# foges/pogs

Hardware: AMD Instinct MI355X
Metric: admm_iterations_per_sec_dense_lasso_fp32 (per-GPU shard, summed over GPUs) (higher is better)
Workload: dtype f32

## Files before the change

pogs_amd/csrc/dense_iter.h:

```cpp

template <typename T, typename Tag>
void DenseSolver<T, Tag>::load_problem(const FnHost &f, const FnHost &g, const SolveParams &p) {
  load_functions(f, g);
  bool all_cheap = true, all_logistic = true;
  if (tmode_) {
    all_logistic = false;
    all_cheap = all_h(g, n_, [](int h) { return is_cheap_prox(h); });
  } else {
    all_cheap = all_h(f, m_, [](int h) { return is_cheap_prox(h); });
    all_logistic = all_h(f, m_, [](int h) { return h == kLogistic; });
  }
  fused_now_ = fused_ok_ && (all_cheap || all_logistic);
  fused_logistic_ = fused_now_ && all_logistic && !all_cheap;
  tune_stream_plan<T>(planA_, fused_now_, fused_logistic_, tmode_);
  arm_control(p);
}

template <typename T, typename Tag>
void DenseSolver<T, Tag>::cold_start() {
  reset_iterate();
  spec_valid_ = false;
  exact_mode_ = false;
  colparts_ = 0;
  proj_count_ = 0;
}

template <typename T, typename Tag>
void DenseSolver<T, Tag>::apply_warm_start() {
  if (!warm_pending_) return;
  warm_pending_ = false;
  hipStream_t s = ctx_.stream;
  const T rho = ctl_.rho;
  POGS_HIP_CHECK(hipMemcpyAsync(xtemp_.p, warm_x_.data(), n_ * sizeof(T), hipMemcpyHostToDevice, s));
  POGS_HIP_CHECK(hipMemcpyAsync(ytemp_.p, warm_l_.data(), m_ * sizeof(T), hipMemcpyHostToDevice, s));
  launch_scale_by<T>(n_, static_cast<T>(1), xtemp_.p, e_.p, true, x_[cur_].p, s);
  launch_scale_by<T>(m_, static_cast<T>(1), ytemp_.p, d_.p, true, yt_.p, s);
  if (tmode_) {
    t_mul_n(x_[cur_].p, nullptr, GemvNOp<T>{1, 0, y_[cur_].p}, nullptr);
    t_mul_t(yt_.p, StoreColOp<T>{static_cast<T>(1) / rho, 0, xt_.p, n_}, nullptr);
  } else {
    StreamArgs<T> a = argsA();
    a.xin = x_[cur_].p;
    launch_stream<T, true, false, false, kFull, Tag>(planA_, a, GemvNOp<T>{1, 0, y_[cur_].p}, s);
    gemv_t_partials(yt_.p);
    finish_cols(StoreColOp<T>{static_cast<T>(1) / rho, 0, xt_.p, n_}, nullptr, 0, 0);
  }
  launch_scal<T>(yt_.p, static_cast<T>(-1) / rho, m_, s);
  ctx_.sync();
  xtemp_.zero(s);
  ytemp_.zero(s);
}

template <typename T, typename Tag>
bool DenseSolver<T, Tag>::iteration(unsigned verbose) {
  if (fused_now_) return tmode_ ? iteration_fused_wide(verbose) : iteration_fused(verbose);
  hipStream_t s = ctx_.stream;
  const int nw = cur_ ^ 1;
  const bool multi = multi_;
  const AdmmPreArgs<T> pa = pre_args();
  const double *S_fused = nullptr;
  if (cg_fused_) {
    S_fused = prox_and_project_fused(pa, nw);
  } else {
    launch_admm_pre<T>(pa, s);
    SumJob j[2] = {{ctx_.spart.p, pa.blocks_x, 3, ctx_.S.p + kGapX},
                   {ctx_.spart.p + static_cast<size_t>(pa.blocks_x) * 3, pre_blocks(m_), 3, ctx_.S.p + kGapY}};
    launch_sum_jobs(j, 2, s);
  }
  if (cg_fused_) {
  } else if (use_cgls_) {
    POGS_HIP_CHECK(hipMemcpyAsync(x_[nw].p, x_[cur_].p, n_ * sizeof(T), hipMemcpyDeviceToDevice, s));
    const bool ysync = ysync_ <= 0 || (proj_count_ % static_cast<unsigned long long>(ysync_)) == 0;
    ++proj_count_;
    const int steps = cgls_project(xtemp_.p, ytemp_.p, x_[nw].p, ctl_.proj_tol(), y_[cur_].p, ysync ? nullptr : y_[nw].p);
    if (ysync) {
      StreamArgs<T> a = argsA();
      a.xin = x_[nw].p;
      ctx_.stream_timer.begin(s);
      launch_stream<T, true, false, false, kFull, Tag>(planA_, a,
                                                  ProjTailOp<T>{y_[nw].p, y_[cur_].p, y12_.p, ytemp_.p}, s);
      ctx_.stream_timer.end(s);
      sum_row_scalars(stream_grid<true, false>(planA_, m_), 2, ctx_.S.p + kDYprev2);
      ctx_.stats.matvecs += 1;
    } else {
      if (steps == 0) POGS_HIP_CHECK(hipMemcpyAsync(y_[nw].p, y_[cur_].p, m_ * sizeof(T), hipMemcpyDeviceToDevice, s));
      double *spy = ctx_.spart.p;
      launch_admm_tail<T>(m_, y_[nw].p, y_[cur_].p, y12_.p, ytemp_.p, spy, s);
      SumJob jy{spy, vec_blocks(m_), 2, ctx_.S.p + kDYprev2};
      launch_sum_jobs(&jy, 1, s);
    }
    double *sp2 = ctx_.spart.p + static_cast<size_t>(planA_.grid_max) * 6;
    launch_admm_tail<T>(n_, x_[nw].p, x_[cur_].p, x12_.p, xtemp_.p, sp2, s);
    SumJob jt{sp2, vec_blocks(n_), 2, ctx_.S.p + kDXprev2};
    launch_sum_jobs(&jt, 1, s);
  } else if (tall_) {
    gemv_t_partials(ytemp_.p);
    finish_cols(StoreColOp<T>{1, 0, rhs_.p, n_}, nullptr, kGapY, 3);
    solve_gram_onepass(rhs_.p, xtemp_.p, ProjTailSumColOp<T>{x_[nw].p, x_[cur_].p, x12_.p, xtemp_.p, n_},
                       ctx_.S.p + kDXprev2);
    StreamArgs<T> a = argsA();
    a.xin = x_[nw].p;
    ctx_.stream_timer.begin(s);
    launch_stream<T, true, false, false, kFull, Tag>(planA_, a,
                                                ProjTailOp<T>{y_[nw].p, y_[cur_].p, y12_.p, ytemp_.p}, s);
    ctx_.stream_timer.end(s);
    sum_row_scalars(stream_grid<true, false>(planA_, m_), 2, ctx_.S.p + kDYprev2);
    if (multi) ctx_.dist.allreduce(ctx_.S.p + kDYprev2, 2, s);
  } else {
    t_mul_n(xtemp_.p, nullptr, ResidOp<T>{ytemp_.p, rhs_.p}, nullptr);
    solve_gram_onepass(rhs_.p, static_cast<const T *>(nullptr),
                       ProjTailAddColOp<T>{y_[nw].p, y_[cur_].p, y12_.p, ytemp_.p, tmpn_.p, m_},
                       ctx_.S.p + kDYprev2);
    t_mul_t(tmpn_.p, ProjTailColOp<T>{x_[nw].p, x_[cur_].p, x12_.p, xtemp_.p, n_}, ctx_.S.p + kDXprev2);
  }
  if (!use_cgls_) ctx_.stats.matvecs += 2;
  const double *S = S_fused ? S_fused : ctx_.fetch_scalars();
  ctl_.set_pre(S);
  bool exact = false;
  if (ctl_.set_approx(S, nrmA_)) {
    StreamArgs<T> a = argsA();
    const int grid = stream_grid<true, true>(planA_, srows_);
    if (tmode_) {
      launch_exact_u<T>(m_, y12_.p, yt_.p, y_[cur_].p, zt_scale_, uvec_.p, s);
      a.xin = uvec_.p;
      ctx_.stream_timer.begin(s);
      launch_stream<T, true, true, false, kFull, Tag>(planA_, a, ExactTRowOp<T>{x12_.p, xt_.p, x_[cur_].p, zt_scale_}, s);
      ctx_.stream_timer.end(s);
      sum_row_scalars(grid, 1, ctx_.S.p + kExactS2);
      double *sp = ctx_.spart.p + static_cast<size_t>(planA_.grid_max) * 6;
      launch_reduce_cols<T, ExactTColOp<T>>(colpart_.p, grid, scols_pad_, ExactTColOp<T>{y12_.p, m_}, sp, s);
      SumJob j{sp, reduce_cols_grid(scols_pad_, Vec16<T>::N), 1, ctx_.S.p + kExactR2};
      launch_sum_jobs(&j, 1, s);
    } else {
      a.xin = x12_.p;
      ctx_.stream_timer.begin(s);
      launch_stream<T, true, true, false, kFull, Tag>(planA_, a,
                                                 ExactRowOp<T>{y12_.p, yt_.p, y_[cur_].p, zt_scale_}, s);
      ctx_.stream_timer.end(s);
      sum_row_scalars(grid, 1, ctx_.S.p + kExactR2);
      finish_cols(ExactColOp<T>{x12_.p, xt_.p, x_[cur_].p, zt_scale_, n_}, ctx_.S.p + kExactS2, kExactR2, 1, grid);
    }
    ctx_.stats.matvecs += 1;
    S = ctx_.fetch_scalars();
    ctl_.set_exact(S);
    exact = true;
  }
  const bool stop = ctl_.check_stop(exact);
  log_iteration(verbose);
  if (stop) return true;
  advance(nw);
  return false;
}

template <typename T, typename Tag>
bool DenseSolver<T, Tag>::iteration_fused(unsigned verbose) {
  hipStream_t s = ctx_.stream;
  const int nw = cur_ ^ 1;
  const int by = pre_blocks(m_);
  const int gridC = pre_cols_grid(n_pad_, Vec16<T>::N);
  struct DeferGuard {
    bool &flag;
    DeferGuard(bool &f, bool on) : flag(f) { flag = on; }
    ~DeferGuard() { flag = false; }
  } defer_guard(defer_sums_, true);
  const bool spec = spec_valid_;
  double *pre_part = ctx_.spart.p + sp_pre_off_;
  double *pc_part = pre_part + static_cast<size_t>(by) * 3;
  double *tail = pack_.p ? pack_.p + 2 * static_cast<size_t>(n_pad_) : nullptr;
  const size_t pack_count = 2 * static_cast<size_t>(n_pad_) + 6;
#ifndef POGS_LEAN_F32_NV5
#define POGS_LEAN_F32_NV5 0
#endif
  constexpr bool kLeanType = std::is_same<T, double>::value || (POGS_LEAN_F32_NV5 != 0 && Tag::has(256, 5) && !Tag::windows);
  const bool lean = kLeanType && !multi_ && !exact_mode_ && !mixed_full_;
  int nparts = colparts_ > 0 ? colparts_ : stream2_grid<2>(planA_, m_);
  if (!spec) {
    AdmmPreArgs<T> pa = pre_args();
    pa.n_x = 0;
    pa.partials = pre_part;
    pa.blocks_x = 0;
    launch_admm_pre<T>(pa, s);
    const SumJob jy{pre_part, by, 3, ctx_.S.p + kGapY};
    StreamArgs2<T> a2{A_.p, lda_, m_, n_pad_, nullptr, nullptr, colpart_.p, colpart2_.p, ctx_.spart.p};
    ctx_.stream_timer.begin(s);
    launch_stream2<T, 0, 2, Tag>(planA_, a2, PreAccOp<T>{ytemp_.p, y12_.p, yt_.p, y_[cur_].p, zt_scale_}, s);
    ctx_.stream_timer.end(s);
    nparts = stream2_grid<0>(planA_, m_);
    ctx_.stats.matvecs += 1;
    if (!multi_) {
      sum_now_or_later(jy);
    } else {
      PackJobs pj;
      pj.j[0] = jy; pj.j[1] = jy; pj.njobs = 1;
      launch_pack_cols<T>(colpart_.p, colpart2_.p, nparts, n_pad_, pack_.p, pj, s);
      ctx_.dist.allreduce(pack_.p, pack_count, s);
      ScalarOverlay ov;
      ov.src = tail; ov.slot[0] = kGapY; ov.n[0] = 3;
      launch_apply_overlay(ctx_.S.p, ov, s);
    }
  }
  {
    PreColsArgs<T> pc;
    pc.part0 = colpart_.p; pc.part1 = (lean && spec) ? nullptr : colpart2_.p; pc.nparts = nparts;
    pc.tot64 = pack_.p;
    pc.n = n_; pc.n_pad = n_pad_;
    pc.g = gview();
    pc.x_cur = x_[cur_].p; pc.xt = xt_.p;
    pc.zt_scale = zt_scale_; pc.rho = ctl_.rho; pc.alpha = ctl_.alpha();
    pc.x12 = x12_.p; pc.xtemp = xtemp_.p; pc.rhs = rhs_.p;
    pc.partials = pc_part;
    launch_pre_cols<T>(pc, multi_, s);
    sum_now_or_later(SumJob{pc_part, gridC, 3, ctx_.S.p + kGapX, 4, 0});
    sum_now_or_later(SumJob{pc_part, gridC, 1, ctx_.S.p + kExactS2, 4, 3});
  }
  solve_gram_onepass(rhs_.p, xtemp_.p, ProjTailSumColOp<T>{x_[nw].p, x_[cur_].p, x12_.p, xtemp_.p, n_},
                     ctx_.S.p + kDXprev2);
  {
    StreamArgs2<T> a2{A_.p, lda_, m_, n_pad_, x_[nw].p, x12_.p, colpart_.p, colpart2_.p, ctx_.spart.p};
    ctl_.predict(&rho_pred_, &zs_pred_);
    const bool timed = ctx_.stream_timer.begin(s) != EventTimer::npos;
    int grid = stream2_grid<2>(planA_, m_);
    bool mixed_done = false;
    if constexpr (std::is_same<T, double>::value) {
      if (mixed_pass_) {
        const StreamArgsMixed am{A32_.p, lda32_, m_, n_pad_, static_cast<int>(lda32_), x_[nw].p, x12_.p, colpart_.p, colpart2_.p,
                                 ctx_.spart.p};
        if (fused_logistic_) {
          launch_stream2_mixed(planM_, !lean, am, FusedIterOp<double, true>{y_[nw].p, y_[cur_].p, y12_.p, ytemp_.p, fview(), rho_pred_,
                                                                            ctl_.alpha(), zs_pred_, y12s_.p, ytemps_.p}, s);
        } else {
          launch_stream2_mixed(planM_, !lean, am, FusedIterOp<double, false>{y_[nw].p, y_[cur_].p, y12_.p, ytemp_.p, fview(), rho_pred_,
                                                                             ctl_.alpha(), zs_pred_, y12s_.p, ytemps_.p}, s);
        }
        grid = mixed_grid(planM_, !lean, m_);
        if (timed) ++mixed_timed_;
        mixed_done = true;
      }
    }
    if (mixed_done) {
    } else if (fused_logistic_) {
      FusedIterOp<T, true> op{y_[nw].p, y_[cur_].p, y12_.p, ytemp_.p, fview(), rho_pred_, ctl_.alpha(), zs_pred_,
                              y12s_.p, ytemps_.p};
      if constexpr (kLeanType) {
        if (lean) { launch_stream2<T, 1, 1, Tag>(planA_, a2, op, s); grid = stream2_grid<1, 1>(planA_, m_); }
        else launch_stream2<T, 2, 2, Tag>(planA_, a2, op, s);
      } else {
        launch_stream2<T, 2, 2, Tag>(planA_, a2, op, s);
      }
    } else {
      FusedIterOp<T, false> op{y_[nw].p, y_[cur_].p, y12_.p, ytemp_.p, fview(), rho_pred_, ctl_.alpha(), zs_pred_,
                               y12s_.p, ytemps_.p};
      if constexpr (kLeanType) {
        if (lean) { launch_stream2<T, 1, 1, Tag>(planA_, a2, op, s); grid = stream2_grid<1, 1>(planA_, m_); }
        else launch_stream2<T, 2, 2, Tag>(planA_, a2, op, s);
      } else {
        launch_stream2<T, 2, 2, Tag>(planA_, a2, op, s);
      }
    }
    ctx_.stream_timer.end(s);
    colparts_ = grid;
    const SumJob jd{ctx_.spart.p, grid, 3, ctx_.S.p + kDYprev2, 6, 0};
    const SumJob js{ctx_.spart.p, grid, 3, ctx_.S.p + kSpecGapY, 6, 3};
    if (!multi_) {
      sum_now_or_later(jd);
      sum_now_or_later(js);
    } else {
      PackJobs pj;
      pj.j[0] = jd; pj.j[1] = js; pj.njobs = 2;
      launch_pack_cols<T>(colpart_.p, colpart2_.p, grid, n_pad_, pack_.p, pj, s);
      ctx_.dist.allreduce(pack_.p, pack_count, s);
      ScalarOverlay ov;
      ov.src = tail;
      ov.slot[0] = kDYprev2; ov.n[0] = 3;
      ov.slot[1] = kSpecGapY; ov.n[1] = 3;
      ctx_.set_overlay(ov);
    }
    ctx_.stats.matvecs += 1;
  }
  double S[kNumSlots];
  std::memcpy(S, ctx_.fetch_scalars(), sizeof(S));
  if (spec)
    for (int q = 0; q < 3; ++q) S[kGapY + q] = spec_gap_[q];
  ctl_.set_pre(S);
  bool exact = false;
  bool drop_spec = false;
  if (ctl_.set_approx(S, nrmA_)) {
    if (lean) {
      StreamArgs<T> a = argsA();
      a.xin = x12_.p;
      a.col_partials = colpart2_.p;
      const int g1 = stream_grid<true, true>(planA_, srows_);
      ctx_.stream_timer.begin(s);
      launch_stream<T, true, true, false, kFull, Tag>(planA_, a, ExactRowOp<T>{y12_.p, yt_.p, y_[cur_].p, zt_scale_}, s);
      ctx_.stream_timer.end(s);
      sum_row_scalars(g1, 1, ctx_.S.p + kExactR2);
      finish_cols(ExactColOp<T>{x12_.p, xt_.p, x_[cur_].p, zt_scale_, n_}, ctx_.S.p + kExactS2, kExactR2, 1, g1, colpart2_.p);
      ctx_.stats.matvecs += 1;
      const double *S2 = ctx_.fetch_scalars();
      S[kExactR2] = S2[kExactR2];
      S[kExactS2] = S2[kExactS2];
      exact_mode_ = true;
      drop_spec = true;
    }
    ctl_.set_exact(S);
    exact = true;
  }
  const bool stop = ctl_.check_stop(exact);
  log_iteration(verbose);
  if (stop) return true;
  advance(nw);
  if (!drop_spec && ctl_.rho == rho_pred_ && zt_scale_ == zs_pred_) {
    std::swap(ytemp_, ytemps_);
    std::swap(y12_, y12s_);
    for (int q = 0; q < 3; ++q) spec_gap_[q] = S[kSpecGapY + q];
    spec_valid_ = true;
    ctx_.stats.reserved[0] += 1;
  } else {
    spec_valid_ = false;
    ctx_.stats.reserved[1] += 1;
  }
  return false;
}

template <typename T, typename Tag>
void DenseSolver<T, Tag>::collect_timer() {
  const unsigned long long cnt = collect_timer_head();
  const unsigned long long mixed = std::min(mixed_timed_, cnt);
  mixed_timed_ = 0;
  ctx_.stats.stream_bytes += static_cast<double>(cnt - mixed) * m_ * n_ * sizeof(T) + static_cast<double>(mixed) * m_ * n_ * sizeof(float);
}
```

pogs_amd/csrc/dense_setup.h:

```cpp

template <typename T, typename Tag>
void DenseSolver<T, Tag>::upload(int ord, const void *A, int mem) {
  hipStream_t s = ctx_.stream;
  A_.alloc(static_cast<size_t>(srows_) * lda_);
  const hipMemcpyKind kind = (mem == POGS_AMD_DEVICE) ? hipMemcpyDeviceToDevice : hipMemcpyHostToDevice;
  const char *ae = std::getenv("POGS_AMD_ALIAS_INPUT");
  bool may_alias = mem == POGS_AMD_DEVICE && !(ae && ae[0] == '0') &&
                   (reinterpret_cast<uintptr_t>(A) % 16) == 0;
  if (may_alias) {
    hipPointerAttribute_t attr;
    if (hipPointerGetAttributes(&attr, A) != hipSuccess) {
      (void)hipGetLastError();
      may_alias = false;
    } else {
      may_alias = attr.type == hipMemoryTypeDevice && attr.device == ctx_.device;
    }
  }
  if (tmode_) {
    if (lda_ != static_cast<size_t>(m_)) A_.zero(s);
    if (ord != ROW_MAJ && may_alias && lda_ == static_cast<size_t>(m_)) {
      A_src_ = static_cast<const T *>(A);
    } else if (ord != ROW_MAJ) {
      POGS_HIP_CHECK(hipMemcpy2DAsync(A_.p, lda_ * sizeof(T), A, m_ * sizeof(T), m_ * sizeof(T), n_, kind, s));
    } else {
      DevBuf<T> stage;
      const T *src = static_cast<const T *>(A);
      if (mem != POGS_AMD_DEVICE) {
        stage.alloc(static_cast<size_t>(m_) * n_);
        POGS_HIP_CHECK(hipMemcpyAsync(stage.p, A, static_cast<size_t>(m_) * n_ * sizeof(T), kind, s));
        src = stage.p;
      }
      launch_transpose<T>(src, n_, m_, n_, A_.p, lda_, s);
      ctx_.sync();
    }
  } else if (ord == ROW_MAJ && may_alias && lda_ == static_cast<size_t>(n_)) {
    A_src_ = static_cast<const T *>(A);
  } else if (ord == ROW_MAJ) {
    if (lda_ != static_cast<size_t>(n_)) A_.zero(s);
    POGS_HIP_CHECK(hipMemcpy2DAsync(A_.p, lda_ * sizeof(T), A, n_ * sizeof(T), n_ * sizeof(T), m_, kind, s));
  } else {
    DevBuf<T> stage;
    const T *src = static_cast<const T *>(A);
    if (mem != POGS_AMD_DEVICE) {
      stage.alloc(static_cast<size_t>(m_) * n_);
      POGS_HIP_CHECK(hipMemcpyAsync(stage.p, A, static_cast<size_t>(m_) * n_ * sizeof(T), kind, s));
      src = stage.p;
    }
    if (lda_ != static_cast<size_t>(n_)) A_.zero(s);
    launch_transpose<T>(src, m_, n_, m_, A_.p, lda_, s);
    ctx_.sync();
  }
  ctx_.sync();
}

template <typename T, typename Tag>
void DenseSolver<T, Tag>::alloc_state() {
  hipStream_t s = ctx_.stream;
  const size_t np = n_pad_;
  const size_t mp = m_pad_;
  alloc_iterate(np, mp);
  const size_t kp = std::max<size_t>(np, k_pad_);
  rhs_.alloc(kp); tvec_.alloc(kp); tmpn_.alloc(kp);
  rhs_.zero(s); tvec_.zero(s); tmpn_.zero(s);
  d_.zero(s); e_.zero(s);
  if (tmode_) { uvec_.alloc(mp); uvec_.zero(s); }
  const size_t gmax = std::max<size_t>(planA_.grid_max, mixed_store_ ? mixed_grid_max(planM_) : 0);
  colpart_.alloc(gmax * scols_pad_);
  ensure_xl(planA_, srows_, scols_pad_);
  if (use_cgls_) {
    cg_p_.alloc(np); cg_s_.alloc(np); cg_q_.alloc(m_); cg_r_.alloc(m_); cg_.alloc(kCgNumSlots);
    cg_p_.zero(s); cg_s_.zero(s); cg_.zero(s);
    if (cg_fused_) alloc_cg_fused();
  }
  const char *fe = std::getenv("POGS_AMD_FUSED");
  fused_ok_ = (tall_ || tmode_) && !use_cgls_ && stream2_supported(planA_) && !(fe && fe[0] == '0');
  if (fused_ok_ && tmode_) {
    colpart2_.alloc(static_cast<size_t>(planA_.grid_max) * scols_pad_);
    x12s_.alloc(np); xtemps_.alloc(np);
    x12s_.zero(s); xtemps_.zero(s);
  } else if (fused_ok_) {
    colpart2_.alloc(gmax * np);
    if (multi_) {
      pack_.alloc(2 * np + 8);
      pack_.zero(s);
    }
    y12s_.alloc(m_); ytemps_.alloc(m_);
    y12s_.zero(s); ytemps_.zero(s);
  }
  const size_t vb = vec_blocks(n_) + vec_blocks(m_);
  const size_t r01 = gmax * 6 + std::max<size_t>(4096, vb * 3 + 64);
  sp_pre_off_ = r01;
  sp_tail_off_ = r01 + vb * 3 + static_cast<size_t>(pre_cols_grid(n_pad_, Vec16<T>::N)) * 4 + 64;
  ctx_.ensure_spart(sp_tail_off_ + static_cast<size_t>(ctx_.num_cu) * 32);
  if (mixed_store_) {
    A32_.alloc(static_cast<size_t>(m_) * lda32_);
    const char *mp = std::getenv("POGS_AMD_MIXED_PASS");
    mixed_pass_ = fused_ok_ && !(mp && mp[0] == '0');
    const char *mf = std::getenv("POGS_AMD_MIXED_FULL");
    mixed_full_ = mixed_pass_ && mf && mf[0] == '1';
  }
}

template <typename T, typename Tag>
void DenseSolver<T, Tag>::equilibrate() {
  hipStream_t s = ctx_.stream;
  PhaseTimer pt(s);
  const double mg = static_cast<double>(ctx_.m_global), nn = n_;
  const T ce = static_cast<T>(1e-4) * static_cast<T>(mg + nn) / static_cast<T>(mg);
  const T cd = static_cast<T>(1e-4) * static_cast<T>(mg + nn) / static_cast<T>(nn);
  const int gridACC = stream_grid<false, true>(planA_, srows_);
  const int gridBOTH = stream_grid<true, true>(planA_, srows_);
  StreamArgs<T> a = argsA();
  if (A_src_) a.A = A_src_;
  ctx_.tmark("  eq: start");
  const char *sk_env = std::getenv("POGS_AMD_SK_FULL");
  const bool sk_probe = !(sk_env && sk_env[0] == '1');
  double *mark = sk_probe ? ctx_.S.p + kSkMark : nullptr;
  const T sk_tol = (std::is_same<T, float>::value ? 16 : 64) * std::numeric_limits<T>::epsilon();
  double r_ref = 0, gamma = 0, gamma_prev = 0;
  bool extrapolate = false, was_uniform = false;
  auto sk_uniform = [&](int k, int count) {
    if (!mark || k < 1) return false;
    const double *S = ctx_.fetch_scalars();
    const double r_mean = S[kSkRatio] / count;
    const bool uniform = k >= 2 && S[kSkMark] < k + 1.0 && r_mean > 0.5 && r_mean < 2.0;
    r_ref = r_mean;
    gamma_prev = gamma;
    gamma = r_mean - 1.0;
    if (std::getenv("POGS_AMD_TRACE"))
      std::fprintf(stderr, "[pogs_amd trace]   sk pass %d: gamma %.6e, %s\n", k, r_mean - 1.0, uniform ? "uniform" : "stamped");
    const bool fire = uniform && (std::is_same<T, float>::value || was_uniform);
    was_uniform = uniform;
    return fire;
  };
  auto sk_log_growth = [&](int first, int count) {
    double q = 1.0;
    if (std::is_same<T, double>::value && gamma != 0 && gamma_prev != 0) {
      q = gamma / gamma_prev;
      if (!(q > 0.999 && q < 1.001)) q = 1.0;
    }
    double L = 0, gi = gamma * std::pow(q, first);
    for (int i = 0; i < count; ++i, gi *= q) L += std::log1p(gi);
    return L;
  };
  int k = 0;
  if (tmode_) {
    double *sp = ctx_.spart.p + static_cast<size_t>(planA_.grid_max) * 6;
    launch_fill<T>(d_.p, static_cast<T>(1), m_, s);
    for (; k < 50; ++k) {
      a.xin = d_.p;
      launch_stream<T, true, true, true, kFull, Tag>(planA_, a, SkRowOp<T>{static_cast<T>(mg), ce, e_.p}, s);
      launch_reduce_cols<T, SkColOp<T>>(
          colpart_.p, gridBOTH, scols_pad_,
          SkColOp<T>{static_cast<T>(nn), cd, d_.p, m_, mark, k + 1.0, sk_tol, static_cast<T>(r_ref)}, sp, s);
      SumJob j{sp, reduce_cols_grid(scols_pad_, Vec16<T>::N), 1, ctx_.S.p + kSkRatio};
      launch_sum_jobs(&j, 1, s);
      if (sk_uniform(k, m_)) { extrapolate = true; ++k; break; }
    }
    ctx_.stats.matvecs_init += k;
    if (extrapolate) {
      const double Ld = sk_log_growth(1, 50 - k);
      const double Le = -sk_log_growth(0, 50 - k);
      launch_scal<T>(d_.p, static_cast<T>(std::exp(Ld)), m_, s);
      launch_scal<T>(e_.p, static_cast<T>(std::exp(Le)), n_, s);
    }
  } else {
    launch_stream<T, false, true, true, kFull, Tag>(planA_, a, OnesOp<T>{}, s);
    ctx_.tmark("  eq: first pass");
    finish_cols(SkColOp<T>{static_cast<T>(mg), ce, e_.p, n_}, nullptr, 0, 0, gridACC);
    ctx_.tmark("  eq: first cols");
    for (; k < 50; ++k) {
      a.xin = e_.p;
      if (k < 49) {
        launch_stream<T, true, true, true, kFull, Tag>(planA_, a, SkRowOp<T>{static_cast<T>(nn), cd, d_.p}, s);
        finish_cols(SkColOp<T>{static_cast<T>(mg), ce, e_.p, n_, mark, k + 1.0, sk_tol, static_cast<T>(r_ref)},
                    ctx_.S.p + kSkRatio, 0, 0, gridBOTH);
        if (sk_uniform(k, n_)) { extrapolate = true; ++k; break; }
      } else {
        launch_stream<T, true, false, true, kFull, Tag>(planA_, a, SkRowOp<T>{static_cast<T>(nn), cd, d_.p}, s);
      }
    }
    ctx_.stats.matvecs_init += k + 1;
    if (extrapolate) {
      const double Le = sk_log_growth(1, 49 - k);
      const double Ld = -sk_log_growth(0, 50 - k);
      launch_scal<T>(d_.p, static_cast<T>(std::exp(Ld)), m_, s);
      launch_scal<T>(e_.p, static_cast<T>(std::exp(Le)), n_, s);
    }
  }
  ctx_.tmark("  eq: sk loop");
  launch_sqrt_inplace<T>(d_.p, m_, s);
  launch_sqrt_inplace<T>(e_.p, n_, s);
  const int sgrid = std::min(srows_, ctx_.num_cu * 8);
  const T *src = A_src_ ? A_src_ : A_.p;
  const T *dr = tmode_ ? e_.p : d_.p, *dc = tmode_ ? d_.p : e_.p;
  hipLaunchKernelGGL((scale_de_kernel<T, false>), dim3(sgrid), dim3(256), 0, s, src, static_cast<T *>(nullptr), lda_,
                     srows_, scols_pad_, dr, dc, static_cast<T>(1), ctx_.spart.p, ctx_.spart.p + sgrid);
  sum_row_scalars(sgrid, 1, ctx_.S.p + kFro2);
  launch_max_partials(ctx_.spart.p + sgrid, sgrid, ctx_.S.p + kAmax, s);
  if (multi_) ctx_.dist.allreduce(ctx_.S.p + kFro2, 1, s);
  const double *S = ctx_.fetch_scalars();
  const T normA = static_cast<T>(std::sqrt(S[kFro2])) /
                  std::sqrt(static_cast<T>(std::min<double>(mg, nn)));
  amax_ = S[kAmax] / static_cast<double>(normA);
  hipLaunchKernelGGL((scale_de_kernel<T, true>), dim3(sgrid), dim3(256), 0, s, src, A_.p, lda_, srows_, scols_pad_,
                     dr, dc, static_cast<T>(1) / normA, static_cast<double *>(nullptr),
                     static_cast<double *>(nullptr));
  A_src_ = nullptr;
  const T invs = static_cast<T>(1) / std::sqrt(normA);
  launch_scal<T>(d_.p, invs, m_, s);
  launch_scal<T>(e_.p, invs, n_, s);
  if constexpr (std::is_same<T, double>::value) {
    if (mixed_store_) {
      launch_round_to_f32(A_.p, lda_, A32_.p, lda32_, m_, n_, sgrid, s);
      amax_ *= 1.0 + 1.0 / (1 << 23);
    }
  }
  ctx_.stats.equil_ms = pt.stop_ms();
}

template <typename T, typename Tag>
void DenseSolver<T, Tag>::norm_est() {
  hipStream_t s = ctx_.stream;
  PhaseTimer pt(s);
  std::vector<T> x0(n_pad_, 0);
  rand_uniform_host(x0.data(), n_);
  POGS_HIP_CHECK(hipMemcpyAsync(xtemp_.p, x0.data(), n_pad_ * sizeof(T), hipMemcpyHostToDevice, s));
  ctx_.sync();
  T *xa = xtemp_.p, *xb = rhs_.p;
  const T kTol = static_cast<T>(1e-4);
  T norm_est = 0, last;
  const int grid = stream_grid<true, true>(planA_, srows_);
  unsigned i = 0;
  for (i = 0; tmode_ && i < 50; ++i) {
    last = norm_est;
    t_mul_n(xa, nullptr, StoreNormRowOp<T>{ytemp_.p}, ctx_.S.p + kPowSx2, (i == 0) ? nullptr : ctx_.S.p + kPowX2);
    t_mul_t(ytemp_.p, PowerColOp<T>{xb, n_}, ctx_.S.p + kPowX2);
    const double *S = ctx_.fetch_scalars();
    norm_est = static_cast<T>(std::sqrt(S[kPowX2])) / static_cast<T>(std::sqrt(S[kPowSx2]));
    std::swap(xa, xb);
// ... 123 lines not shown
```

pogs_amd/csrc/dense_solver.h:

```cpp
#pragma once
#include <algorithm>
#include <array>
#include <cmath>
#include <cstdint>
#include <cstdio>
#include <cstdlib>
#include <limits>
#include <thread>

#include "batch_admm.h"
#include "batch_kernels.h"
#include "cg_fused.h"
#include "cg_kernels.h"
#include "engine.h"
#include "fused_cols.h"
#include "gemm.h"
#include "gram_phase.h"
#include "ops.h"
#include "reduce.h"
#include "solo_solver.h"
#include "stream.h"
#include "stream_mixed.h"
#include "vec_kernels.h"

// ... 270 lines not shown
      StreamArgs<T> a = argsA();
      a.xin = xin; a.xin_add = xin_add; a.xin_nrm2 = x_nrm2;
      ctx_.stream_timer.begin(s);
      launch_stream<T, true, false, false, kFull, Tag>(planA_, a, op, s);
      ctx_.stream_timer.end(s);
      if (RowOp::NS > 0 && scalar_out) sum_row_scalars(stream_grid<true, false>(planA_, srows_), RowOp::NS, scalar_out);
      return;
    }
    StreamArgs<T> a = argsA();
    ctx_.stream_timer.begin(s);
    launch_stream<T, false, true, false, kFull, Tag>(planA_, a, VecCoefOp<T>{xin, xin_add, x_nrm2}, s);
    ctx_.stream_timer.end(s);
    double *sp = ctx_.spart.p + static_cast<size_t>(planA_.grid_max) * 6;
    launch_reduce_cols<T, RowAsColOp<T, RowOp>>(colpart_.p, stream_grid<false, true>(planA_, srows_), scols_pad_,
                                                RowAsColOp<T, RowOp>{op, m_}, sp, s);
    if (RowOp::NS > 0 && scalar_out) {
      SumJob j{sp, reduce_cols_grid(scols_pad_, Vec16<T>::N), RowOp::NS, scalar_out};
      launch_sum_jobs(&j, 1, s);
    }
  }
  template <typename ColOp>
  void t_mul_t(const T *u, const ColOp &op, double *scalar_out) {
    hipStream_t s = ctx_.stream;
    if (!tmode_) {
      gemv_t_partials(u);
      finish_cols(op, scalar_out, 0, 0);
      return;
    }
    StreamArgs<T> a = argsA();
    a.xin = u;
    ctx_.stream_timer.begin(s);
    launch_stream<T, true, false, false, kFull, Tag>(planA_, a, ColAsRowOp<T, ColOp>{op}, s);
    ctx_.stream_timer.end(s);
    if (ColOp::NS > 0 && scalar_out) sum_row_scalars(stream_grid<true, false>(planA_, srows_), ColOp::NS, scalar_out);
  }

  template <typename ColOp>
  void finish_cols(const ColOp &op, double *colop_scalar_out, int yslot, int yslot_count,
                   int nparts_override = -1, const T *partials_src = nullptr) {
    hipStream_t s = ctx_.stream;
    const T *colpart = partials_src ? partials_src : colpart_.p;
    const int nparts = nparts_override > 0 ? nparts_override : stream_grid<false, true>(planA_, m_);
    double *sp = ctx_.spart.p + static_cast<size_t>(planA_.grid_max) * 6;
    if (!multi_) {
      launch_reduce_cols<T, ColOp>(colpart, nparts, n_pad_, op, sp, s);
    } else {
      launch_reduce_cols<T, StoreColOp<T>>(colpart, nparts, n_pad_, StoreColOp<T>{1, 0, tmpn_.p, n_}, sp, s);
      if (yslot_count > 0) ctx_.dist.allreduce2(tmpn_.p, n_pad_, ctx_.S.p + yslot, yslot_count, s);
      else ctx_.dist.allreduce(tmpn_.p, n_pad_, s);
      launch_reduce_cols<T, ColOp>(tmpn_.p, 1, n_pad_, op, sp, s);
    }
    if (ColOp::NS > 0 && colop_scalar_out) {
      SumJob j{sp, reduce_cols_grid(n_pad_, Vec16<T>::N), ColOp::NS, colop_scalar_out};
      sum_now_or_later(j);
    }
  }

  void sum_now_or_later(const SumJob &j) {
    if (defer_sums_) ctx_.queue_sum(j);
    else launch_sum_jobs(&j, 1, ctx_.stream);
  }

  void gemv_t_partials(const T *u) {
    StreamArgs<T> a = argsA();
    ctx_.stream_timer.begin(ctx_.stream);
    launch_stream<T, false, true, false, kFull, Tag>(planA_, a, GemvTOp<T>{1, u}, ctx_.stream);
    ctx_.stream_timer.end(ctx_.stream);
  }

  void sum_row_scalars(int grid, int ns, double *out) {
    SumJob j{ctx_.spart.p, grid, ns, out};
    launch_sum_jobs(&j, 1, ctx_.stream);
  }

  void equilibrate();

  void norm_est();

  void norm_est_gram(T *G, size_t ld);

  void norm_est_gram_wide(T *G, size_t ld);

  void factor();

  template <typename TailOp>
  void solve_gram(const T *rhs, const T *add, const TailOp &tail, double *tail_scalars);

  template <typename TailColOp>
  void solve_gram_onepass(const T *rhs, const T *add, const TailColOp &tail, double *tail_scalars);

  int cgls_project(const T *x0, const T *y0, T *x, T tol, const T *Ax_warm, T *yacc = nullptr);

  void alloc_cg_fused();
  const double *cg_loop_fused(T *x, const T *xprev, const T *ycur, T *ynew, int ahead_steps, int max_steps, double tol,
                              const double *pre_part, int *enqueued);
  const double *project_cg_fused(int nw, bool ysync, int ahead, int max_steps, double tol, const double *pre_part,
                                 int *enqueued);
  const double *prox_and_project_fused(const AdmmPreArgs<T> &pa0, int nw);
  void project_start_fused(double tol);

  void load_problem(const FnHost &f, const FnHost &g, const SolveParams &p) override;
  void cold_start() override;
  void apply_warm_start() override;
  bool iteration(unsigned verbose) override;
  void collect_timer() override;
  void print_solver_line(int status) override {
    std::printf("POGS-AMD dense/%s: status %d, iter %u, init %.3e s, loop %.3e s\n", cg_fused_ ? "cgls-fused" : use_cgls_ ? "cgls" : "direct",
                status, ctl_.k, ctx_.stats.t_init_s, ctx_.stats.t_loop_s);
  }

  bool iteration_fused(unsigned verbose);

  bool iteration_fused_wide(unsigned verbose);

  void log_iteration(unsigned verbose) {
    const bool was_deferring = defer_sums_;
    defer_sums_ = false;
    B::log_iteration(verbose);
    defer_sums_ = was_deferring;
  }

  int n_pad_ = 0, k_ = 0, k_pad_ = 0;
  bool tall_ = true, use_cgls_ = false;
  double amax_ = 0;
  bool defer_sums_ = false;
  size_t sp_pre_off_ = 0, sp_tail_off_ = 0;
  double spec_gap_[3] = {0, 0, 0};
  bool tmode_ = false;
  int m_pad_ = 0, srows_ = 0, scols_pad_ = 0;
  DevBuf<T> xl_buf_;
  DevBuf<T> uvec_;
  DevBuf<T> x12s_, xtemps_;
  DevBuf<T> cg_p_, cg_s_, cg_q_, cg_r_;
  DevBuf<double> cg_;
  bool cg_fused_ = false;
  int cg_pred_ = 1;
  DevBuf<double> cgf_rec_;
  size_t cgo_q_ = 0, cgo_p_ = 0, cgo_x_ = 0, cgo_s_ = 0, cgo_s0_ = 0, cgo_pre_ = 0, cgo_close_ = 0;
  std::vector<size_t> cgf_events_;
  size_t lda_ = 0;
  StreamPlan planA_, planW_;
  bool mixed_store_ = false, mixed_pass_ = false;
  bool mixed_full_ = false;
  MixedPlan planM_;
  DevBuf<float> A32_;
  size_t lda32_ = 0;
  unsigned long long mixed_timed_ = 0;
  const T *A_src_ = nullptr;
  T *Wp_ = nullptr, *Up_ = nullptr;
  DevBuf<T> A_, fac_, colpart_, colpart2_, y12s_, ytemps_;
  DevBuf<double> pack_;
  bool fused_ok_ = false, fused_now_ = false, fused_logistic_ = false, spec_valid_ = false;
  bool exact_mode_ = false;
  int colparts_ = 0;
  T rho_pred_ = 1, zs_pred_ = 1;
  int ysync_ = 16;
  unsigned long long proj_count_ = 0;
  DevBuf<T> rhs_, tvec_, tmpn_;
};

#include "dense_setup.h"
#include "dense_factor.h"
#include "dense_cg_fused.h"
#include "dense_iter.h"
#include "dense_wide.h"
#include "dense_batch.h"

}

template <typename T, typename Tag>
SolverBase *make_dense_solver_t(int ord, size_t m, size_t n, const void *A, int mem, const PogsAmdOptions *opt,
                                const PogsAmdDist *dist) {
  return new DenseSolver<T, Tag>(ord, m, n, A, mem, opt, dist);
}

}
```

pogs_amd/csrc/engine.h:

```cpp
#pragma once
#include <hip/hip_runtime.h>

#include <algorithm>
#include <chrono>
#include <cmath>
#include <cstdio>
#include <cstdlib>
#include <limits>
#include <cstring>
#include <memory>
#include <mutex>
#include <string>
#include <vector>

#include "../../include/pogs_amd.h"
#include "common.h"
#include "dist.h"
#include "vec_kernels.h"

namespace pogs_amd {

inline double wall_s() {
  return std::chrono::duration<double>(std::chrono::steady_clock::now().time_since_epoch()).count();
}
// ... 54 lines not shown
      if (dropped_[i]) continue;
      float ms = 0;
      if (hipEventElapsedTime(&ms, ev_[i].first, ev_[i].second) == hipSuccess) tot += ms;
      ++kept;
    }
    if (count) *count += kept;
    used_ = 0;
    return tot;
  }
  ~EventTimer() {
    for (auto &p : ev_) { (void)hipEventDestroy(p.first); (void)hipEventDestroy(p.second); }
  }
 private:
  bool on_ = false, active_ = false;
  unsigned every_ = 1;
  unsigned long long calls_ = 0;
  size_t used_ = 0;
  std::vector<std::pair<hipEvent_t, hipEvent_t>> ev_;
  std::vector<char> dropped_;
};

struct PhaseTimer {
  hipEvent_t a = nullptr, b = nullptr;
  hipStream_t s;
  explicit PhaseTimer(hipStream_t st) : s(st) {
    POGS_HIP_CHECK(hipEventCreate(&a));
    POGS_HIP_CHECK(hipEventCreate(&b));
    POGS_HIP_CHECK(hipEventRecord(a, s));
  }
  double stop_ms() {
    POGS_HIP_CHECK(hipEventRecord(b, s));
    POGS_HIP_CHECK(hipEventSynchronize(b));
    float ms = 0;
    POGS_HIP_CHECK(hipEventElapsedTime(&ms, a, b));
    return ms;
  }
  ~PhaseTimer() {
    if (a) (void)hipEventDestroy(a);
    if (b) (void)hipEventDestroy(b);
  }
};

struct CtxResources {
  hipStream_t stream = nullptr;
  double *host = nullptr;
  int device = -1;
};
inline std::mutex &ctx_pool_mutex() { static std::mutex *m = new std::mutex; return *m; }
inline std::vector<CtxResources> &ctx_pool() { static auto *v = new std::vector<CtxResources>; return *v; }
struct Ctx {
  int device = 0;
  int num_cu = 256;
  hipStream_t stream = nullptr;
  DistComm dist;
  size_t m_global = 0;
  DevBuf<double> S;
  struct HostMirror { double *p = nullptr; } S_host;
  DevBuf<double> spart;
  size_t spart_cap = 0;
  EventTimer stream_timer;
  PogsAmdStats stats;

  void init(int dev, int profile) {
    if (dev >= 0) POGS_HIP_CHECK(hipSetDevice(dev));
    POGS_HIP_CHECK(hipGetDevice(&device));
    hipDeviceProp_t prop;
    POGS_HIP_CHECK(hipGetDeviceProperties(&prop, device));
    num_cu = prop.multiProcessorCount > 0 ? prop.multiProcessorCount : 256;
    {
      std::lock_guard<std::mutex> lock(ctx_pool_mutex());
      auto &pool = ctx_pool();
      for (size_t i = 0; i < pool.size(); ++i)
        if (pool[i].device == device) {
          stream = pool[i].stream;
          S_host.p = pool[i].host;
          pool.erase(pool.begin() + static_cast<long>(i));
          break;
        }
    }
    if (!stream) {
      POGS_HIP_CHECK(hipStreamCreateWithFlags(&stream, hipStreamNonBlocking));
      POGS_HIP_CHECK(hipHostMalloc(reinterpret_cast<void **>(&S_host.p), (kNumSlots + 1) * sizeof(double),
                                   hipHostMallocMapped | hipHostMallocCoherent));
    }
    S.alloc(kNumSlots);
    S.zero(stream);
    pub_counter.alloc(1);
    pub_counter.zero(stream);
    std::memset(S_host.p, 0, (kNumSlots + 1) * sizeof(double));
    {
      void *dp = nullptr;
      poll_fetch = true;
      if (hipHostGetDevicePointer(&dp, S_host.p, 0) == hipSuccess && dp) S_host_dev = static_cast<double *>(dp);
      else poll_fetch = false;
    }
    std::memset(&stats, 0, sizeof(stats));
    stream_timer.enable(profile != 0);
    stream_timer.set_every(profile > 1 ? static_cast<unsigned>(profile) : 1u);
  }
  void ensure_spart(size_t count) {
    if (count > spart_cap) {
      POGS_HIP_CHECK(hipStreamSynchronize(stream));
      spart.alloc(count);
      spart_cap = count;
    }
  }
  void queue_sum(const SumJob &j) {
    if (npending == kMaxSumJobs) flush_sums();
    pending[npending++] = j;
  }
  void flush_sums() {
    if (npending) launch_sum_jobs(pending, npending, stream);
    npending = 0;
  }
  void set_overlay(const ScalarOverlay &ov) { overlay = ov; }
  const double *wait_publish(unsigned long long want) {
    unsigned long long *seqp = reinterpret_cast<unsigned long long *>(S_host.p + kNumSlots);
    unsigned spins = 0, idle_seen = 0, checks = 0;
    double t_wait0 = 0;
    while (__atomic_load_n(seqp, __ATOMIC_ACQUIRE) != want) {
      if (++spins == (1u << 14)) {
        spins = 0;
        if (dist.active() && (++checks & 255u) == 0) {
          const double now = wall_s();
          if (t_wait0 == 0) t_wait0 = now;
          const char *ae = dist.async_error();
          if (ae[0] || now - t_wait0 > coll_timeout_s()) {
            const std::string why = ae[0] ? std::string("RCCL reported: ") + ae
                                          : "no progress for " + std::to_string(static_cast<int>(coll_timeout_s())) +
                                                " s inside a collective (a peer rank did not join it)";
            dist.abort();
            poisoned = true;
            throw Error("row-sharded solve aborted: " + why);
          }
        }
        const hipError_t q = hipStreamQuery(stream);
        if (q == hipSuccess) {
          if (__atomic_load_n(seqp, __ATOMIC_ACQUIRE) == want) break;
          if (++idle_seen >= 3) {
            POGS_HIP_CHECK(hipMemcpy(S_host.p, S.p, kNumSlots * sizeof(double), hipMemcpyDeviceToHost));
            poll_fetch = false;
            return S_host.p;
          }
        } else if (q != hipErrorNotReady) {
          POGS_HIP_CHECK(q);
        }
      }
#if defined(__x86_64__)
      __builtin_ia32_pause();
#endif
    }
    return S_host.p;
  }
  const double *fetch_scalars() {
    const ScalarOverlay ov = overlay;
    overlay = ScalarOverlay();
    if (!poll_fetch) {
      flush_sums();
      launch_apply_overlay(S.p, ov, stream);
      POGS_HIP_CHECK(hipMemcpyAsync(S_host.p, S.p, kNumSlots * sizeof(double), hipMemcpyDeviceToHost, stream));
      POGS_HIP_CHECK(hipStreamSynchronize(stream));
      return S_host.p;
    }
    const unsigned long long want = ++fetch_seq;
    if (npending) {
      launch_sum_publish(pending, npending, S.p, kNumSlots, S_host_dev,
                         reinterpret_cast<unsigned long long *>(S_host_dev + kNumSlots), want, pub_counter.p, stream, ov);
      npending = 0;
    } else {
      launch_publish_scalars(S.p, kNumSlots, S_host_dev, reinterpret_cast<unsigned long long *>(S_host_dev + kNumSlots),
                             want, stream, ov);
    }
    return wait_publish(want);
  }
  static double coll_timeout_s() {
    static const double v = [] {
      const char *e = std::getenv("POGS_AMD_COLL_TIMEOUT_S");
      const double t = e ? std::atof(e) : 300.0;
      return t > 0 ? t : 300.0;
    }();
    return v;
  }
  bool poll_fetch = true;
  ScalarOverlay overlay;
  SumJob pending[kMaxSumJobs];
  int npending = 0;
  DevBuf<unsigned> pub_counter;
  unsigned long long fetch_seq = 0;
  double *S_host_dev = nullptr;
  void sync() {
    flush_sums();
    POGS_HIP_CHECK(hipStreamSynchronize(stream));
  }
  void tmark(const char *label) {
    static const bool on = std::getenv("POGS_AMD_TRACE") != nullptr;
    if (!on) return;
    const double t1 = wall_s();
    POGS_HIP_CHECK(hipStreamSynchronize(stream));
    const double t2 = wall_s();
    const PoolCounters pc = DevicePool::get().counters(device);
    std::fprintf(stderr, "[pogs_amd trace] %-28s host +%8.3f ms, drain +%8.3f ms | pool: +%llu malloc %.3f ms, +%llu reuse, "
                 "+%llu free %.3f ms\n", label, (t1 - tmark_last) * 1e3, (t2 - t1) * 1e3,
                 pc.mallocs - tmark_pool.mallocs, pc.malloc_ms - tmark_pool.malloc_ms, pc.reuses - tmark_pool.reuses,
                 pc.frees - tmark_pool.frees, pc.free_ms - tmark_pool.free_ms);
    tmark_pool = pc;
    tmark_last = wall_s();
  }
  double tmark_last = 0;
  PoolCounters tmark_pool;
  bool poisoned = false;
  unsigned long long coll_mark = 0;
  void on_entry() { coll_mark = dist.collectives(); }
  void on_error() {
    if (dist.active() && dist.collectives() != coll_mark) {
      dist.abort();
      poisoned = true;
    }
  }
  ~Ctx() {
    if (!stream) return;
    DeviceGuard guard(device);
    const bool healthy = !poisoned && hipStreamSynchronize(stream) == hipSuccess;
    if (healthy) {
      std::lock_guard<std::mutex> lock(ctx_pool_mutex());
      CtxResources r;
      r.stream = stream;
      r.host = S_host.p;
      r.device = device;
      ctx_pool().push_back(r);
    } else {
      (void)hipStreamDestroy(stream);
      if (S_host.p) (void)hipHostFree(S_host.p);
    }
  }
};

#define POGS_HD __host__ __device__
#if defined(__HIP_DEVICE_COMPILE__)
#define POGS_SAY_RHO(fmt, ...) ((void)0)
#else
#define POGS_SAY_RHO(fmt, ...) do { if (say_rho) std::printf(fmt, __VA_ARGS__); } while (0)
#endif
POGS_HD inline float ctl_abs(float v) { return fabsf(v); }
POGS_HD inline double ctl_abs(double v) { return fabs(v); }
POGS_HD inline float ctl_sqrt(float v) { return sqrtf(v); }
POGS_HD inline double ctl_sqrt(double v) { return sqrt(v); }
POGS_HD inline float ctl_pow(float a, float b) { return powf(a, b); }
POGS_HD inline double ctl_pow(double a, double b) { return pow(a, b); }
template <typename T> POGS_HD inline T ctl_min(T a, T b) { return b < a ? b : a; }
template <typename T> POGS_HD inline T ctl_max(T a, T b) { return a < b ? b : a; }

template <typename T>
struct AdmmControl {
  T abs_tol = 0, rel_tol = 0;
  unsigned max_iter = 0;
  bool adaptive_rho = true, gap_stop = false;
  T rho0 = 1;
  size_t m_glob = 0, n = 0;
  T rho = 1, delta = 0, xi = 1;
  unsigned k = 0, kd = 0, ku = 0;
  T prev_nrm_r = 0;
  T nrm_r = 0, nrm_s = 0, gap = 0, eps_gap = 0, eps_pri = 0, eps_dua = 0;
  bool converged = false, finished = false;
  unsigned exact_iters = 0, rho_updates = 0;
  bool say_rho = false;
  T sqrtn_atol = 0, sqrtm_atol = 0, sqrtmn_atol = 0;

  static constexpr double kAlphaD = 1.7;
  POGS_HD T alpha() const { return static_cast<T>(kAlphaD); }

  void reset() {
    rho = rho0;
    delta = static_cast<T>(1.05);
    xi = 1;
    k = kd = ku = 0;
    prev_nrm_r = std::numeric_limits<T>::max();
    converged = finished = false;
    exact_iters = rho_updates = 0;
    sqrtn_atol = std::sqrt(static_cast<T>(n)) * abs_tol;
    sqrtm_atol = std::sqrt(static_cast<T>(m_glob)) * abs_tol;
    sqrtmn_atol = std::sqrt(static_cast<T>(m_glob + n)) * abs_tol;
  }

  POGS_HD void set_pre(const double *S) {
    gap = ctl_abs(static_cast<T>(S[kGapX] + S[kGapY]));
    const T nz = static_cast<T>(ctl_sqrt(S[kWX2] + S[kWY2]));
    const T nz12 = static_cast<T>(ctl_sqrt(S[kHX2] + S[kHY2]));
    const T ny12 = static_cast<T>(ctl_sqrt(S[kHY2]));
    const T nx = static_cast<T>(ctl_sqrt(S[kWX2]));
    eps_gap = sqrtmn_atol + rel_tol * nz * nz12;
    eps_pri = sqrtm_atol + rel_tol * ny12;
    eps_dua = rho * (sqrtn_atol + rel_tol * nx);
  }
  POGS_HD T proj_tol() const {
    T tol = static_cast<T>(1e-2) * ctl_pow(ctl_min(prev_nrm_r, static_cast<T>(1)), static_cast<T>(0.5));
    return ctl_max(tol, static_cast<T>(1e-8));
  }
  POGS_HD bool set_approx(const double *S, T nrmA) {
    nrm_s = rho * (nrmA * static_cast<T>(ctl_sqrt(S[kDYprev2])) + static_cast<T>(ctl_sqrt(S[kDXprev2])));
    nrm_r = nrmA * static_cast<T>(ctl_sqrt(S[kDX12])) + static_cast<T>(ctl_sqrt(S[kDY12]));
    return nrm_r < 10 * eps_pri && nrm_s < 10 * eps_dua;
  }
  POGS_HD void set_exact(const double *S) {
    nrm_r = static_cast<T>(ctl_sqrt(S[kExactR2]));
    nrm_s = rho * static_cast<T>(ctl_sqrt(S[kExactS2]));
    ++exact_iters;
  }
  POGS_HD bool check_stop(bool exact) {
    converged = exact && nrm_r < eps_pri && nrm_s < eps_dua && (!gap_stop || gap < eps_gap);
    if (converged || k == max_iter - 1) {
      finished = true;
      return true;
    }
    return false;
  }
  POGS_HD T adapt() {
    T scale = 1;
    const T kDeltaMin = static_cast<T>(1.05), kGamma = static_cast<T>(1.01), kTau = static_cast<T>(0.8);
    const T kRhoMin = static_cast<T>(1e-4), kRhoMax = static_cast<T>(1e4), kKappa = static_cast<T>(0.9);
    const T kOne = 1, kZero = 0;
    if (adaptive_rho) {
      const unsigned kRhoUpdateFreq = 50u;
      const T kRhoChangeMax = static_cast<T>(1.5), kRhoChangeMin = static_cast<T>(0.67);
      const T kImbalanceThresh = static_cast<T>(10);
      if (k > 0 && k % kRhoUpdateFreq == 0 && eps_pri > kZero && eps_dua > kZero) {
        const T pri_n = nrm_r / eps_pri, dua_n = nrm_s / eps_dua;
// ... 271 lines not shown
```

Measured before the change: 1539.

## Speculatively launch next iteration's column pre-pass while waiting on scalar fetch

Splits the scalar fetch into enqueue and await steps. Between them it launches the next iteration's pre-columns kernel into spare buffers, using the predicted rho and z-scale, so the GPU has work while the host waits on the convergence scalars. If the prediction holds, the buffers are swapped and the next iteration skips its pre-columns launch. This costs extra device buffers and wasted work on mispredicted iterations, and adds correctness risk from sharing the partials buffer.

```diff
diff --git a/pogs_amd/csrc/dense_iter.h b/pogs_amd/csrc/dense_iter.h
--- a/pogs_amd/csrc/dense_iter.h
+++ b/pogs_amd/csrc/dense_iter.h
@@ -20,6 +20,7 @@
 void DenseSolver<T, Tag>::cold_start() {
   reset_iterate();
   spec_valid_ = false;
+  colspec_valid_ = false;
   exact_mode_ = false;
   colparts_ = 0;
   proj_count_ = 0;
@@ -209,7 +210,8 @@
     pc.zt_scale = zt_scale_; pc.rho = ctl_.rho; pc.alpha = ctl_.alpha();
     pc.x12 = x12_.p; pc.xtemp = xtemp_.p; pc.rhs = rhs_.p;
     pc.partials = pc_part;
-    launch_pre_cols<T>(pc, multi_, s);
+    if (!colspec_valid_) launch_pre_cols<T>(pc, multi_, s);
+    colspec_valid_ = false;
     sum_now_or_later(SumJob{pc_part, gridC, 3, ctx_.S.p + kGapX, 4, 0});
     sum_now_or_later(SumJob{pc_part, gridC, 1, ctx_.S.p + kExactS2, 4, 3});
   }
@@ -278,7 +280,21 @@
     ctx_.stats.matvecs += 1;
   }
   double S[kNumSlots];
-  std::memcpy(S, ctx_.fetch_scalars(), sizeof(S));
+  const unsigned long long want = ctx_.enqueue_publish();
+  const bool cols_ahead = colspec_on_ && ctl_.k != ctl_.max_iter - 1;
+  if (cols_ahead) {
+    PreColsArgs<T> pc;
+    pc.part0 = colpart_.p; pc.part1 = lean ? nullptr : colpart2_.p; pc.nparts = colparts_;
+    pc.tot64 = nullptr;
+    pc.n = n_; pc.n_pad = n_pad_;
+    pc.g = gview();
+    pc.x_cur = x_[nw].p; pc.xt = xtemp_.p;
+    pc.zt_scale = zs_pred_; pc.rho = rho_pred_; pc.alpha = ctl_.alpha();
+    pc.x12 = x12s_.p; pc.xtemp = xtemps_.p; pc.rhs = rhs_.p;
+    pc.partials = pc_part;
+    launch_pre_cols<T>(pc, false, s);
+  }
+  std::memcpy(S, ctx_.await_publish(want), sizeof(S));
   if (spec)
     for (int q = 0; q < 3; ++q) S[kGapY + q] = spec_gap_[q];
   ctl_.set_pre(S);
@@ -314,6 +330,11 @@
     std::swap(y12_, y12s_);
     for (int q = 0; q < 3; ++q) spec_gap_[q] = S[kSpecGapY + q];
     spec_valid_ = true;
+    if (cols_ahead) {
+      std::swap(x12_, x12s_);
+      std::swap(xtemp_, xtemps_);
+      colspec_valid_ = true;
+    }
     ctx_.stats.reserved[0] += 1;
   } else {
     spec_valid_ = false;
diff --git a/pogs_amd/csrc/dense_setup.h b/pogs_amd/csrc/dense_setup.h
--- a/pogs_amd/csrc/dense_setup.h
+++ b/pogs_amd/csrc/dense_setup.h
@@ -86,6 +86,12 @@
     }
     y12s_.alloc(m_); ytemps_.alloc(m_);
     y12s_.zero(s); ytemps_.zero(s);
+    const char *cs = std::getenv("POGS_AMD_COLSPEC");
+    colspec_on_ = !multi_ && !(cs && cs[0] == '0');
+    if (colspec_on_) {
+      x12s_.alloc(np); xtemps_.alloc(np);
+      x12s_.zero(s); xtemps_.zero(s);
+    }
   }
   const size_t vb = vec_blocks(n_) + vec_blocks(m_);
   const size_t r01 = gmax * 6 + std::max<size_t>(4096, vb * 3 + 64);
diff --git a/pogs_amd/csrc/dense_solver.h b/pogs_amd/csrc/dense_solver.h
--- a/pogs_amd/csrc/dense_solver.h
+++ b/pogs_amd/csrc/dense_solver.h
@@ -446,6 +446,7 @@
   DevBuf<double> pack_;
   bool fused_ok_ = false, fused_now_ = false, fused_logistic_ = false, spec_valid_ = false;
   bool exact_mode_ = false;
+  bool colspec_on_ = false, colspec_valid_ = false;
   int colparts_ = 0;
   T rho_pred_ = 1, zs_pred_ = 1;
   int ysync_ = 16;
diff --git a/pogs_amd/csrc/engine.h b/pogs_amd/csrc/engine.h
--- a/pogs_amd/csrc/engine.h
+++ b/pogs_amd/csrc/engine.h
@@ -230,15 +230,22 @@
     }
     return S_host.p;
   }
-  const double *fetch_scalars() {
+  const double *fetch_scalars() { return await_publish(enqueue_publish()); }
+  const double *await_publish(unsigned long long want) {
+    if (want == 0) {
+      POGS_HIP_CHECK(hipStreamSynchronize(stream));
+      return S_host.p;
+    }
+    return wait_publish(want);
+  }
+  unsigned long long enqueue_publish() {
     const ScalarOverlay ov = overlay;
     overlay = ScalarOverlay();
     if (!poll_fetch) {
       flush_sums();
       launch_apply_overlay(S.p, ov, stream);
       POGS_HIP_CHECK(hipMemcpyAsync(S_host.p, S.p, kNumSlots * sizeof(double), hipMemcpyDeviceToHost, stream));
-      POGS_HIP_CHECK(hipStreamSynchronize(stream));
-      return S_host.p;
+      return 0;
     }
     const unsigned long long want = ++fetch_seq;
     if (npending) {
@@ -249,7 +256,7 @@
       launch_publish_scalars(S.p, kNumSlots, S_host_dev, reinterpret_cast<unsigned long long *>(S_host_dev + kNumSlots),
                              want, stream, ov);
     }
-    return wait_publish(want);
+    return want;
   }
   static double coll_timeout_s() {
     static const double v = [] {
```

New measurement: 1528. Within noise of the previous version (-0.7%).
